# xiaojino/RUArt

Hardware: AMD Instinct MI355X
Metric: VQA samples/sec fwd+bwd (B=64, q=30, ocr=100) (higher is better)
Workload: dtype f16 MFMA + block-scaled fp8 (e4m3) MFMA correction, f32 accumulate / residual stream; 1 GPU; RUArt training step, synthetic ST-VQA-shaped batch: B=64/GPU, q=30 words, 100 OCR items, 36 objects, bert-base 12x768 frozen, SDNet trunk fwd+bwd, Adamax; global_batch=64, real_wordpieces_per_batch=42738, parallelism=dp1, mode=train

## Files before the change

### ruart_amd/bert.py

```python
import ctypes
import os
from ctypes import c_void_p

import numpy as np
import torch
import torch.nn as nn

from . import hip

LONG_BLOCK = 128
ROW_PAD = 256


def _np(x):
    return x.detach().cpu().numpy() if isinstance(x, torch.Tensor) else np.asarray(x)


def split_f16c(x, lo_shift=None, hi_shift=None):
    hi = x.to(torch.float16)
    lo = x - hi.to(torch.float32)
    sa_lo, sa_hi, _, _ = hip.f16c_shifts()
    lo_shift = sa_lo if lo_shift is None else lo_shift
    hi_shift = sa_hi if hi_shift is None else hi_shift
    pair = torch.cat([lo * float(2.0 ** lo_shift), x * float(2.0 ** hi_shift)], 1).clamp_(-448.0, 448.0)
# ... 137 lines not shown


def train_layer_split(opt, n_layers):
    if "bert_train_layers" not in opt:
        return 0
    n = opt["bert_train_layers"]
    if isinstance(n, bool) or not isinstance(n, (int, np.integer)) or n < 1 or n > n_layers:
        raise ValueError("opt['bert_train_layers'] = %r: the number of trained top layers is an integer in 1 .. %d" % (n, n_layers))
    if "LOCK_BERT" in opt:
        raise ValueError("opt['bert_train_layers'] trains encoder layers, LOCK_BERT freezes all of them: a conf has one or the other")
    if str(opt.get("bert_train_gemm", "x3")) != "16":
        raise ValueError("opt['bert_train_layers'] cuts the 16-bit trainable encoder only: it needs opt['bert_train_gemm'] = '16' (got %r)"
                         % (opt.get("bert_train_gemm", "x3"),))
    if opt.get("bert_no_pack", False):
        raise ValueError("opt['bert_train_layers'] runs on the packed token stream: it does not combine with opt['bert_no_pack']")
    return int(n_layers) - int(n)


class LowerLayers:

    def __init__(self, weights, k):
        if not 0 < k <= weights.n_layers:
            raise ValueError("the lower part holds 1 .. %d layers, not %d" % (weights.n_layers, k))
        self.full = weights
        self.cfg, self.device, self.precision = weights.cfg, weights.device, weights.precision
        self.dtype, self.tdtype, self.corr8, self.ln_fold = weights.dtype, weights.tdtype, weights.corr8, weights.ln_fold
        self.hidden, self.n_layers = weights.hidden, int(k)
        m = hip.BertModelC()
        ctypes.memmove(ctypes.byref(m), ctypes.byref(weights.c_model), ctypes.sizeof(m))
        m.n_layers = int(k)
        self.c_model = m
        if self.ln_fold:
            self.ln2_g_all, self.ln2_b_all = weights.ln2_g_all[:k], weights.ln2_b_all[:k]


class PackedTokens:

    def __init__(self, groups, device=None, pack=True, mfma_long=True, window=512, max_positions=None, dedup=False):
        ids_l, pos_l, len_l, bias_l = [], [], [], []
        self.group_index = []
        base = 0
        for ids, mask in groups:
            ids = _np(ids).astype(np.int64)
            mask = _np(mask).astype(bool)
            N, L = ids.shape
            if max_positions is not None and min(L, window) > max_positions:
                raise ValueError("BERT input rows of %d word pieces need %d position embeddings, the checkpoint has %d"
                                 % (L, min(L, window), max_positions))
            keep = mask if pack else np.ones_like(mask)
            if (keep.sum(1) == 0).any():
                raise ValueError("a BERT input row has no attendable token")
            nw = (L + window - 1) // window
            canon = None
            if dedup and nw == 1 and N > 1:
                key = np.ascontiguousarray(np.where(keep, ids, -1))
                _, first, inv = np.unique(key.view(np.dtype((np.void, key.dtype.itemsize * L))).reshape(-1), return_index=True, return_inverse=True)
                canon = first[inv.reshape(-1)]
                if (canon == np.arange(N)).all():
                    canon = None
                else:
                    keep = keep & (canon == np.arange(N))[:, None]
            if nw == 1:
                lens = keep.sum(1).astype(np.int64)
                lens = lens[lens > 0] if canon is not None else lens
            else:
                padded = np.zeros((N, nw * window), dtype=bool)
                padded[:, :L] = keep
                lens = padded.reshape(N, nw, window).sum(2).reshape(-1).astype(np.int64)
                lens = lens[lens > 0]
            flat = keep.reshape(-1)
            idx = np.full(N * L, -1, dtype=np.int64)
            idx[flat] = base + np.arange(int(flat.sum()))
            idx = idx.reshape(N, L)
            self.group_index.append(idx if canon is None else idx[canon])
            ids_l.append(ids.reshape(-1)[flat])
            pos_l.append(np.broadcast_to(np.arange(L) % window, (N, L)).reshape(-1)[flat])
            len_l.append(lens)
            if not pack:
                bias_l.append(np.where(mask.reshape(-1), 0.0, -10000.0).astype(np.float32))
            base += int(flat.sum())
        lens = np.concatenate(len_l)
        T = int(lens.sum())
        Tp = (T + ROW_PAD - 1) // ROW_PAD * ROW_PAD
        cu = np.zeros(len(lens) + 1, dtype=np.int64)
        np.cumsum(lens, out=cu[1:])
        seq_of = np.repeat(np.arange(len(lens)), lens)
        blk, lblk = self._plan_blocks(lens, cu, mfma_long)
        nb, nlb = blk.shape[1], lblk.shape[1]
        host = np.zeros(2 * Tp + 2 * T + 4 * nb + 4 * nlb, dtype=np.int32)
        host[0:T] = np.concatenate(ids_l)
        host[Tp:Tp + T] = np.concatenate(pos_l)
        host[2 * Tp:2 * Tp + T] = cu[seq_of]
        host[2 * Tp + T:2 * Tp + 2 * T] = cu[seq_of + 1]
        host[2 * Tp + 2 * T:2 * Tp + 2 * T + 4 * nb] = blk.reshape(-1)
        host[2 * Tp + 2 * T + 4 * nb:] = lblk.reshape(-1)
        self.T, self.Tp, self.n_blocks, self.n_long_blocks = T, Tp, nb, nlb
        self.n_seq = len(lens)
        self.max_len = int(lens.max())
        self.max_pos = int(host[Tp:Tp + T].max()) + 1 if T else 0
        self.sum_len_sq = float((lens.astype(np.float64) ** 2).sum())
        self.host = host
        self.bias_host = np.concatenate(bias_l) if not pack else None
        self.buf = None
        if device is not None:
            self.bind(device)

    _DEVICE_FIELDS = ("buf", "ids", "pos", "tok_lo", "tok_hi", "blk", "lblk", "key_bias", "c_batch", "_layers", "_event", "_set", "_train_plan",
                      "_emb_sorts", "last_rows")

    def prepare_embedding_sorts(self):
        if getattr(self, "_emb_sorts_host", None) is None:
            from .batch import _sort_ids
            T, Tp = self.T, self.Tp
            sorts = [_sort_ids(ids) for ids in (self.host[0:T], self.host[Tp:Tp + T])]
            self._emb_sorts_host = (np.concatenate([a for srt in sorts for a in srt]).astype(np.int32), [[len(a) for a in srt] for srt in sorts])
        return self._emb_sorts_host

    def train_plan(self, device):
        plan = getattr(self, "_train_plan", None)
        if plan is None or plan["device"] != device:
            T, Tp, nb, nlb = self.T, self.Tp, self.n_blocks, self.n_long_blocks
            o = 2 * Tp + 2 * T
            blk = self.host[o:o + 4 * nb].reshape(4, nb)
            lblk = self.host[o + 4 * nb:o + 4 * nb + 4 * nlb].reshape(4, nlb)
            own = (blk[0] == blk[2]) & (blk[1] == blk[3]) & ((blk[1] - blk[0]) <= 64)
            win = blk[:2, own]
            ch = [tuple(int(v) for v in blk[:, i]) for i in np.nonzero(~own)[0]]
            for i in range(nlb):
                q0, q1, k0, k1 = (int(v) for v in lblk[:, i])
                ch += [(a, min(a + 64, q1), k0, k1) for a in range(q0, q1, 64)]
            ch.sort()
            ok = all(q1 - q0 <= 64 and (q0 - k0) % 64 == 0 and k0 <= q0 < q1 <= k1 for q0, q1, k0, k1 in ch)
            idx = {c[0]: i for i, c in enumerate(ch)}
            ok = ok and all(k0 in idx and (q0 - k0) // 64 == i - idx[k0] for i, (q0, q1, k0, k1) in enumerate(ch))
            arr = np.array([c + (idx.get(c[2], 0),) for c in ch], dtype=np.int32).reshape(-1, 5).T.copy()
            both = torch.from_numpy(np.concatenate([win.reshape(-1), arr.reshape(-1)]).astype(np.int32)).to(device)
            nw, nc = win.shape[1], arr.shape[1]
            plan = {"device": device, "ok": bool(ok), "n_win": nw, "n_chunks": nc,
                    "win": [both[i * nw:(i + 1) * nw] for i in range(2)],
                    "chunks": [both[2 * nw + i * nc:2 * nw + (i + 1) * nc] for i in range(5)]}
            self._train_plan = plan
        return plan

    def embedding_sorts(self, device):
        if getattr(self, "_emb_sorts", None) is None:
            flat, sizes = self.prepare_embedding_sorts()
            dev = torch.from_numpy(flat).to(device, non_blocking=True)
            out, o = [], 0
            for group in sizes:
                views = []
                for n in group:
                    views.append(dev[o:o + n])
                    o += n
                out.append(tuple(views))
            self._emb_sorts = out
        return self._emb_sorts

    def __getstate__(self):
        return {k: v for k, v in self.__dict__.items() if k not in self._DEVICE_FIELDS}

    def __setstate__(self, state):
        self.__dict__.update(state)
        self.buf = None

    def bind(self, device, host_tensor=None):
        T, Tp, nb, nlb = self.T, self.Tp, self.n_blocks, self.n_long_blocks
        dev = (host_tensor if host_tensor is not None else torch.from_numpy(self.host)).to(device, non_blocking=True)
        self.buf = dev
        o = 0
        self.ids = dev[o:o + Tp]; o += Tp
        self.pos = dev[o:o + Tp]; o += Tp
        self.tok_lo = dev[o:o + T]; o += T
        self.tok_hi = dev[o:o + T]; o += T
        self.blk = [dev[o + i * nb:o + (i + 1) * nb] for i in range(4)]
        o += 4 * nb
        self.lblk = [dev[o + i * nlb:o + (i + 1) * nlb] for i in range(4)]
        self.key_bias = None
        if self.bias_host is not None:
            self.key_bias = torch.from_numpy(self.bias_host).to(device)
        b = hip.BertBatchC()
        b.n_tokens, b.n_rows, b.n_blocks = T, Tp, nb
        b.ids, b.pos_ids = self.ids.data_ptr(), self.pos.data_ptr()
        b.blk_q0, b.blk_q1, b.blk_k0, b.blk_k1 = [t.data_ptr() for t in self.blk]
        b.tok_lo, b.tok_hi = self.tok_lo.data_ptr(), self.tok_hi.data_ptr()
        b.key_bias = self.key_bias.data_ptr() if self.key_bias is not None else None
        b.n_long_blocks = nlb
        b.lblk_q0, b.lblk_q1, b.lblk_k0, b.lblk_k1 = [t.data_ptr() if nlb else None for t in self.lblk]
        b.n_last_rows, b.last_rows = 0, None
        self.c_batch = b
        return self

    def set_last_rows(self, rows_dev):
        self.last_rows = rows_dev
        self.c_batch.n_last_rows = int(rows_dev.numel())
        self.c_batch.last_rows = rows_dev.data_ptr()

    @staticmethod
    def _plan_blocks(lens, cu, mfma_long=True):
        S = len(lens)
        short, long_ = [], []
        s = 0
        while s < S:
            if lens[s] > 64:
                tgt, step = (long_, LONG_BLOCK) if mfma_long else (short, 64)
                for q0 in range(int(cu[s]), int(cu[s + 1]), step):
                    tgt.append((q0, min(q0 + step, int(cu[s + 1])), int(cu[s]), int(cu[s + 1])))
                s += 1
                continue
            e = int(np.searchsorted(cu, cu[s] + 64, side="right")) - 1
            while e > s + 1 and (lens[s:e] > 64).any():
                e -= 1
            e = max(e, s + 1)
            short.append((int(cu[s]), int(cu[e]), int(cu[s]), int(cu[e])))
            s = e
        def arr(x):
            return np.array(x, dtype=np.int32).reshape(-1, 4).T.copy()
        return arr(short), arr(long_)


class _Buffers:

    def __init__(self):
        self.layers = None
        self.ws = None
        self.stats = None

    def get(self, w, Tp):
        lib = hip.kernels()
        es = 4 if w.dtype == hip.DT_F32 else 2
        need_l = w.n_layers * Tp * w.hidden * es
        if self.layers is None or self.layers.numel() < need_l or self.layers.device != w.device:
            self.layers = torch.zeros(need_l, dtype=torch.uint8, device=w.device)
        fold = getattr(w, "ln_fold", False)
        need_w = int((lib.ruart_bert_workspace_bytes_folded if fold else lib.ruart_bert_workspace_bytes)(ctypes.byref(w.c_model), Tp))
        if self.ws is None or self.ws.numel() < need_w or self.ws.device != w.device:
            self.ws = torch.zeros(need_w, dtype=torch.uint8, device=w.device)
        if fold:
            need_s = w.n_layers * Tp * 2
            if self.stats is None or self.stats.numel() < need_s or self.stats.device != w.device:
                self.stats = torch.zeros(need_s, dtype=torch.float32, device=w.device)
        return self.layers[:need_l].view(w.tdtype).view(w.n_layers, Tp, w.hidden), self.ws, need_w

    def stats_for(self, w, Tp):
        return self.stats[:w.n_layers * Tp * 2].view(w.n_layers, Tp, 2)


_buffers = _Buffers()


def bert_encode(weights, packed, buffers=None):
    lib = hip.kernels()
    if getattr(packed, "max_pos", 0) > weights.cfg["max_position_embeddings"]:
        raise ValueError("the packed stream addresses %d position embeddings, the checkpoint has %d"
                         % (packed.max_pos, weights.cfg["max_position_embeddings"]))
    buffers = buffers or _buffers
    layers, ws, ws_bytes = buffers.get(weights, packed.Tp)
    if getattr(weights, "ln_fold", False):
        stats = buffers.stats_for(weights, packed.Tp)
        lib.ruart_bert_forward_folded(ctypes.byref(weights.c_model), ctypes.byref(packed.c_batch), layers, stats, ws, ws_bytes, hip.stream_ptr())
        layers._ln = (stats, weights.ln2_g_all, weights.ln2_b_all)
        return layers
    lib.ruart_bert_forward(ctypes.byref(weights.c_model), ctypes.byref(packed.c_batch), layers, ws, ws_bytes, hip.stream_ptr())
    return layers


def layer_outputs(layers, n_last=None):
    ln = getattr(layers, "_ln", None)
    if ln is None:
        return layers
    stats, g, b = ln
    return (layers - stats[:, :, 0:1]) * stats[:, :, 1:2] * g[:, None, :] + b[:, None, :]


from .ops import _ABL_SKIP


class _PoolMix(torch.autograd.Function):

    @staticmethod
    def forward(ctx, layer_w, layers, span_start, span_len, dst_row, n_rows, dtype_code, span_start_last=None, ln_stats=None, ln_g=None,
                ln_b=None):
        lib = hip.kernels()
        NL, Tp, H = layers.shape
        W = span_start.numel()
        out = torch.zeros(n_rows, H, dtype=torch.float32, device=layers.device)
        lw = layer_w.detach().to(torch.float32).contiguous()
        if W > 0 and "pool" not in _ABL_SKIP:
            if ln_stats is not None:
                lib.ruart_bert_pool_mix_ln(layers, Tp * H, H, NL, ln_stats, Tp, ln_g, ln_b, span_start, span_start_last, span_len, dst_row, lw,
                                           out, H, W, H, hip.stream_ptr())
            else:
                lib.ruart_bert_pool_mix(layers, Tp * H, H, dtype_code, NL, span_start, span_start_last, span_len, dst_row, lw, out, H, W, H,
                                        hip.stream_ptr())
        ctx.save_for_backward(layers, span_start, span_len, dst_row, span_start_last, ln_stats, ln_g, ln_b)
        ctx.dtype_code = dtype_code
        return out

    @staticmethod
    def backward(ctx, grad_out):
        lib = hip.kernels()
        layers, span_start, span_len, dst_row, span_start_last, ln_stats, ln_g, ln_b = ctx.saved_tensors
        NL, Tp, H = layers.shape
        W = span_start.numel()
        g = torch.zeros(NL, dtype=torch.float32, device=layers.device)
        if W > 0 and "pool" not in _ABL_SKIP:
            grad_out = grad_out.contiguous()
            partial = torch.empty(W * NL, dtype=torch.float32, device=layers.device)
            if ln_stats is not None:
                lib.ruart_bert_pool_mix_ln_bwd(layers, Tp * H, H, NL, ln_stats, Tp, ln_g, ln_b, span_start, span_start_last, span_len, dst_row,
                                               grad_out, H, partial, g, W, H, hip.stream_ptr())
            else:
                lib.ruart_bert_pool_mix_bwd(layers, Tp * H, H, ctx.dtype_code, NL, span_start, span_start_last, span_len, dst_row, grad_out, H,
                                            partial, g, W, H, hip.stream_ptr())
        return g, None, None, None, None, None, None, None, None, None, None


def word_spans(packed, group, offsets, word_mask, offsets_arr=None):
    wm = _np(word_mask).astype(bool)
    N, Lw = wm.shape
    if offsets_arr is None:
        offsets_arr = np.zeros((N, Lw, 2), dtype=np.int64)
        for n, row in enumerate(offsets):
            if len(row) and not isinstance(row[0], (list, tuple)):
                continue
            k = min(len(row), Lw)
            if k:
                offsets_arr[n, :k] = np.asarray(row[:k], dtype=np.int64)
    offsets_arr = _np(offsets_arr)
    st, ed = offsets_arr[..., 0], offsets_arr[..., 1]
    sel = wm & (ed > st)
    n_idx, j_idx = np.nonzero(sel)
    gidx = packed.group_index[group]
    s, e = st[sel], ed[sel]
    start = gidx[n_idx, s]
    last = gidx[n_idx, e - 1]
    if (start < 0).any() or (last - start != e - s - 1).any():
        raise ValueError("a word's piece span touches a masked BERT position; encode this batch with pack=False")
    return start.astype(np.int32), (e - s).astype(np.int32), (n_idx * Lw + j_idx).astype(np.int32), N * Lw


class Bert(nn.Module):

    def __init__(self, opt, device=None):
        super().__init__()
        import json
        import os
        self.opt = opt
        self.linear_combine = "BERT_LINEAR_COMBINE" in opt
        self.bert_dim, self.bert_layer = (1024, 24) if "BERT_LARGE" in opt else (768, 12)
        self._device = torch.device(device if device is not None else "cuda")
        if "bert_state" in opt:
            state, cfg = opt["bert_state"], opt["bert_config"]
        else:
            key = "BERT_large_model_file" if "BERT_LARGE" in opt else "BERT_model_file"
            d = os.path.join(opt.get("datadir", ""), opt[key])
            with open(os.path.join(d, "bert_config.json")) as f:
                cfg = json.load(f)
            state = torch.load(os.path.join(d, "pytorch_model.bin"), map_location="cpu")
        if cfg["hidden_size"] != self.bert_dim or cfg["num_hidden_layers"] != self.bert_layer:
            raise ValueError("BERT checkpoint is %dx%d, conf expects %dx%d" % (cfg["num_hidden_layers"], cfg["hidden_size"],
                                                                              self.bert_layer, self.bert_dim))
        from . import precision_of
        precision = precision_of(opt, cfg["hidden_size"] if cfg["intermediate_size"] % 256 == 0 else 1)
        fold = bool(int(opt.get("bert_ln_fold", os.environ.get("RUART_LN_FOLD", 1))))
        if int(opt.get("bert_tail_cus", os.environ.get("RUART_TAIL_CUS", 0)) or 0) > 0:
            fold = False
        if precision != "fp16c":
            fold = False
        self.weights = BertEncoderWeights(state, cfg, self._device, precision, ln_fold=fold)
        self.n_frozen = train_layer_split(opt, cfg["num_hidden_layers"])
        self.bert_model = None
        self._source = (state, cfg)
        self.pack = not opt.get("bert_no_pack", False)
        self._opt_prefetch_cus = opt.get("bert_prefetch_cus", 224 if precision == "fp16c" else 0)
        self._init_pipeline()
        tail = opt.get("bert_tail_cus", os.environ.get("RUART_TAIL_CUS", 0))
        self.weights.c_model.tail_cus = max(0, int(tail))

    def unlock(self):
        from .bert_train import BertModelTrainable
        if not self.pack:
            raise NotImplementedError("the trainable encoder runs on the packed token stream (bert_no_pack is for the frozen path)")
        state, cfg = self._source
        mode = str(self.opt.get("bert_train_gemm", "x3"))
        if mode == "16" and cfg["hidden_size"] % 256 == 0 and cfg["intermediate_size"] % 256 == 0:
            from .bert_train16 import BertModelTrainable16
            self.bert_model = BertModelTrainable16(state, cfg, self._device)
            self.bert_model.accurate_forward = bool(self.opt.get("bert_train_accurate_fwd", True))
            if self.n_frozen and self.weights.precision != "fp16c":
                raise ValueError("opt['bert_train_layers']: the frozen lower layers run on the fp16c kernels (bert_precision = %r)"
                                 % (self.weights.precision,))
            if self.n_frozen:
                self._lower_weights = LowerLayers(self.weights, self.n_frozen)
                self.bert_model.freeze_below(self.n_frozen, self.lower_layers_for)
        else:
            if self.n_frozen:
                raise ValueError("opt['bert_train_layers'] needs hidden / intermediate sizes that are multiples of 256")
            self.bert_model = BertModelTrainable(state, cfg, self._device, gemm="16" if mode in ("16", "16gemm") else "x3")
        self._source = None

    def lock(self):
        if self.opt.get("bert_frozen_dropout"):
            from .bert_train import BertModelTrainable
            state, cfg = self._source
            if (self.weights.precision in ("fp16c", "fp16", "bf16") and cfg["hidden_size"] % 256 == 0
                    and cfg["intermediate_size"] % 256 == 0):
                from .bert_train16 import BertModelTrainable16
                model = BertModelTrainable16(state, cfg, self._device)
            else:
                model = BertModelTrainable(state, cfg, self._device, gemm="x3")
            for p in model.parameters():
                p.requires_grad_(False)
            self.__dict__["_dropout_model"] = model
        self._source = None

    def _frozen_dropout_active(self):
        return self.training and self.__dict__.get("_dropout_model") is not None

    def _init_pipeline(self):
        self._bufsets = [_Buffers(), _Buffers()]
        self._pending = None
        self._in_use = 1
        cus = os.environ.get("RUART_PREFETCH_CUS", self._opt_prefetch_cus)
        self._pf_cus = cus if cus == "auto" else int(cus)
        self._pf_streams = {}

    def plan_prefetch_cus(self, n_rows):
        cfg = self.weights.cfg
        H, I = cfg["hidden_size"], cfg["intermediate_size"]
        rt = -(-int(n_rows) // 256)
        prods = ((3 * H // 256, 1.0), (H // 256, 1.0), (I // 256, 1.0), (H // 256, I / float(H)))
        best = None
        for c in range(208, 249, 8):
            cost = sum(w * -(-rt * nt // c) for nt, w in prods)
            if best is None or cost < best[0] - 1e-9:
                best = (cost, c)
        return best[1]

    def prefetch_cus(self, packed=None):
        if self.training:
            if self._pf_cus == "auto":
                if packed is None:
                    return 240
                self._pf_cus = self.plan_prefetch_cus(packed.Tp)
            return self._pf_cus
        return int(os.environ.get("RUART_PREFETCH_CUS_EVAL", 0))

    def prefetch(self, packed, after_stream=None):
        lower = self.runs_ahead()
        if getattr(packed, "_layers", None) is not None or (getattr(self, "bert_model", None) is not None and not lower) \
                or self._frozen_dropout_active():
            return
        weights = self._lower_weights if lower else self.weights
        dev = self._device
        cus = self.prefetch_cus(packed)
        st = self._pf_streams.get(cus)
        if st is None or st.device != dev:
            epr = int(os.environ.get("RUART_ENCODER_PRIORITY", 0))
            st = self._pf_streams[cus] = hip.cu_masked_stream(cus, dev) if cus > 0 else torch.cuda.Stream(device=dev, priority=epr)
        if after_stream is not None:
            st.wait_stream(after_stream)
        elif getattr(self, "_pickup_event", None) is not None:
            st.wait_event(self._pickup_event)
        else:
            st.wait_stream(torch.cuda.current_stream(dev))
        if getattr(self, "_last_pf_event", None) is not None:
            st.wait_event(self._last_pf_event)
        if self._pending is not None and self._pending is not packed:
            self._pending._layers = None
        self._pending = packed
        with torch.cuda.stream(st):
            packed._set = self._in_use ^ 1
            packed._layers = bert_encode(weights, packed, self._bufsets[packed._set])
            packed._event = self._last_pf_event = st.record_event()

    def close(self, destroy=None):
        if destroy is None:
            destroy = os.environ.get("RUART_DESTROY_STREAMS") == "1"
        if self._pending is not None:
            self._pending._layers = None
            self._pending = None
        if not destroy:
            for st in getattr(self, "_pf_streams", {}).values():
                st.synchronize()
            return
        streams, self._pf_streams = getattr(self, "_pf_streams", {}), {}
        self._last_pf_event = None
        for st in streams.values():
            hip.destroy_stream(st)

    def layers_for(self, packed):
        if getattr(self, "bert_model", None) is not None:
            return self.bert_model(packed, training=self.training)
        if self._frozen_dropout_active():
            with torch.no_grad():
                model = self.__dict__["_dropout_model"]
                fast = model.layers_nograd(packed, training=True) if hasattr(model, "layers_nograd") else None
                return fast if fast is not None else model(packed, training=True)
        return self._pickup(packed, self.weights)

    def runs_ahead(self):
        model = getattr(self, "bert_model", None)
        return bool(model is not None and self.n_frozen and self.training and self.opt.get("bert_train_prefetch", True)
                    and model.mixed_pass(True))

    def lower_layers_for(self, packed):
        return self._pickup(packed, self._lower_weights)

    def _pickup(self, packed, weights):
        layers = getattr(packed, "_layers", None)
        if layers is not None:
            torch.cuda.current_stream(self._device).wait_event(packed._event)
            packed._layers = None
            self._pending = None
            self._in_use = packed._set
            self._pickup_event = torch.cuda.current_stream(self._device).record_event()
            return layers
        pend = self._pending
        if pend is None or getattr(pend, "_layers", None) is None or pend._set != self._in_use ^ 1:
            self._in_use ^= 1
        self._pickup_event = torch.cuda.current_stream(self._device).record_event()
        return bert_encode(weights, packed, self._bufsets[self._in_use])

    def encode(self, groups):
        packed = PackedTokens(groups, self._device, pack=self.pack, mfma_long=self.weights.dtype != hip.DT_F32,
                              max_positions=self.weights.cfg["max_position_embeddings"])
        if getattr(self, "bert_model", None) is not None:
            return packed, self.bert_model(packed, training=self.training)
        return packed, bert_encode(self.weights, packed)

    def pool_mix(self, packed, layers, group, offsets, word_mask, layer_w, offsets_arr=None):
        s, n, d, rows = word_spans(packed, group, offsets, word_mask, offsets_arr)
        dev = self._device
        desc = torch.from_numpy(np.concatenate([s, n, d])).to(dev)
        W = len(s)
        if getattr(self, "bert_model", None) is not None:
            from .bert_train import pool_mix
            out = pool_mix(layer_w, layers, desc[:W], desc[W:2 * W], desc[2 * W:], rows)
        else:
            ln = getattr(layers, "_ln", None) or (None, None, None)
            out = _PoolMix.apply(layer_w, layers, desc[:W], desc[W:2 * W], desc[2 * W:], rows, hip.dtype_code(layers), None, *ln)
        N, Lw = word_mask.shape
        return out.view(N, Lw, self.weights.hidden)

    def forward(self, x_bert, x_bert_mask, x_bert_offset, x_mask, device=None):
        bs = getattr(self, "opt", {}).get("BERT_MAX_BatchSize")
        N = x_bert.shape[0]
        if bs and N > bs:
            parts = []
            for st in range(0, N, int(bs)):
                ed = min(st + int(bs), N)
                off = x_bert_offset[st:ed] if x_bert_offset is not None else None
                parts.append(self.forward(x_bert[st:ed], x_bert_mask[st:ed], off, x_mask[st:ed], device=device))
            return [torch.cat([p[i] for p in parts], 0) for i in range(len(parts[0]))]
        packed, layers = self.encode([(x_bert, x_bert_mask)])
        outs = []
        eye = torch.eye(self.weights.n_layers, device=self._device)
        for l in range(self.weights.n_layers):
            outs.append(self.pool_mix(packed, layers, 0, x_bert_offset, x_mask, eye[l]))
        return outs
```

### ruart_amd/csrc/bert_kernels.hip

```cpp
#include <stdlib.h>
#include "common.h"
#include <type_traits>
#include "ruart_hip.h"

#define MAXG 4

template <typename TOut>
struct RowStorePlain {
  TOut* out;
  __device__ __forceinline__ void operator()(int c, f32x4_t o) const { store4(out + c, o); }
};
struct RowStoreSplit {
  float* o32;
  f16_t* o16;
  unsigned char* o8;
  int H;
  __device__ __forceinline__ void operator()(int c, f32x4_t o) const {
    store4(o32 + c, o);
    store_split4(o16 + c, o8 + c, H, o);
  }
};

template <typename Store>
__device__ __forceinline__ void ln_row_finish(f32x4_t (&v)[MAXG], int H, int lane, const float* gamma, const float* beta,
// ... 1098 lines not shown
  g_attn_split_hpg = heads_per_workgroup;
  return 0;
}

extern "C" int ruart_bert_embed_ln(const int* ids, const int* pos, const float* word_emb, const float* pos_emb,
                                   const float* type_emb, const float* gamma, const float* beta, float eps, void* out, int ldo,
                                   int out_dtype, int rows, int H, void* stream) {
  RUART_ENTRY();
  if (H % 4 || H > 256 * MAXG || rows <= 0 || (ldo & 3)) return (int)hipErrorInvalidValue;
  const dim3 grid(ceil_div(rows, 4)), block(256);
  if (out_dtype == RUART_DT_BF16)
    hipLaunchKernelGGL(embed_ln_kernel<bf16_t>, grid, block, 0, (hipStream_t)stream, ids, pos, word_emb, pos_emb, type_emb, gamma, beta, eps, (bf16_t*)out, ldo, rows, H);
  else if (out_dtype == RUART_DT_F16)
    hipLaunchKernelGGL(embed_ln_kernel<f16_t>, grid, block, 0, (hipStream_t)stream, ids, pos, word_emb, pos_emb, type_emb, gamma, beta, eps, (f16_t*)out, ldo, rows, H);
  else
    hipLaunchKernelGGL(embed_ln_kernel<float>, grid, block, 0, (hipStream_t)stream, ids, pos, word_emb, pos_emb, type_emb, gamma, beta, eps, (float*)out, ldo, rows, H);
  RUART_CHECK_LAUNCH();
  return 0;
}

extern "C" int ruart_bert_attention(const void* qkv, int ld, void* ctx, int ldc, int dtype, int H, int n_heads, int n_blocks,
                                    const int* blk_q0, const int* blk_q1, const int* blk_k0, const int* blk_k1,
                                    const int* tok_lo, const int* tok_hi, const float* key_bias, int n_long_blocks,
                                    const int* lblk_q0, const int* lblk_q1, const int* lblk_k0, const int* lblk_k1, void* stream) {
  RUART_ENTRY();
  if (n_heads * 64 != H || n_blocks < 0 || n_long_blocks < 0 || n_blocks + n_long_blocks <= 0) return (int)hipErrorInvalidValue;
  if (n_long_blocks > 0 && dtype == RUART_DT_F32) return (int)hipErrorInvalidValue;
  hipStream_t st = (hipStream_t)stream;
  if (dtype == RUART_DT_F32) {
    if (n_blocks > 0) {
      hipLaunchKernelGGL(attn_varlen_kernel<float>, dim3(n_blocks, n_heads), dim3(64), 0, st, (const float*)qkv, ld, (float*)ctx, ldc, H, blk_q0, blk_q1, blk_k0, blk_k1, tok_lo, tok_hi, key_bias);
      RUART_CHECK_LAUNCH();
    }
    return 0;
  }
  if (n_blocks > 0) {
    const dim3 grid = attn_grid(n_blocks, n_heads), block(256);
    if (dtype == RUART_DT_BF16)
      hipLaunchKernelGGL(attn_flash_kernel<bf16_t>, grid, block, 0, st, (const bf16_t*)qkv, ld, (bf16_t*)ctx, ldc, H, blk_q0, blk_q1, blk_k0, blk_k1, tok_lo, key_bias);
    else
      hipLaunchKernelGGL(attn_flash_kernel<f16_t>, grid, block, 0, st, (const f16_t*)qkv, ld, (f16_t*)ctx, ldc, H, blk_q0, blk_q1, blk_k0, blk_k1, tok_lo, key_bias);
    RUART_CHECK_LAUNCH();
  }
  if (n_long_blocks > 0) {
    const dim3 grid = attn_grid(n_long_blocks, n_heads), block(256);
    if (dtype == RUART_DT_BF16)
      hipLaunchKernelGGL(attn_flash_long_kernel<bf16_t>, grid, block, 0, st, (const bf16_t*)qkv, ld, (bf16_t*)ctx, ldc, H, lblk_q0, lblk_q1, lblk_k0, lblk_k1, key_bias, n_long_blocks);
    else
      hipLaunchKernelGGL(attn_flash_long_kernel<f16_t>, grid, block, 0, st, (const f16_t*)qkv, ld, (f16_t*)ctx, ldc, H, lblk_q0, lblk_q1, lblk_k0, lblk_k1, key_bias, n_long_blocks);
    RUART_CHECK_LAUNCH();
  }
  return 0;
}

struct PoolLN {
  const float2* stats;
  size_t stats_stride;
  const float* g;
  const float* b;
};
__global__ __launch_bounds__(256) void pool_mix_cols_ln_kernel(const float* __restrict__ layers, size_t layer_stride, int ldl, int NL,
                                                               const int* __restrict__ span_start, const int* __restrict__ span_start_last,
                                                               const int* __restrict__ span_len, const int* __restrict__ dst_row,
                                                               const float* __restrict__ wl, float* __restrict__ out, int ldo, int W, int H,
                                                               PoolLN ln) {
  constexpr int LB = 6;
  const int w = blockIdx.x;
  const int st = span_start[w], n = span_len[w];
  const int st_last = span_start_last ? span_start_last[w] : st;
  const float inv = 1.0f / (float)n;
  const int col = threadIdx.x * 4;
  f32x4_t acc = {0.f, 0.f, 0.f, 0.f};
  auto body = [&](auto two_tag) {
    constexpr bool TWO = decltype(two_tag)::value;
    for (int lb = 0; lb < NL; lb += LB) {
      f32x4_t v[LB][TWO ? 2 : 1], g[LB], be[LB];
      float2 sa[LB][TWO ? 2 : 1];
      float wgt[LB];
#pragma unroll
      for (int j = 0; j < LB; ++j) {
        const int l = min(lb + j, NL - 1);
        wgt[j] = (lb + j < NL) ? wl[l] : 0.f;
        const int r0 = (l == NL - 1 ? st_last : st);
        const float* base = layers + (size_t)l * layer_stride + (size_t)r0 * ldl + col;
        v[j][0] = load4_stream(base);
        sa[j][0] = ln.stats[(size_t)l * ln.stats_stride + r0];
        if (TWO) {
          v[j][TWO ? 1 : 0] = load4_stream(base + (size_t)ldl);
          sa[j][TWO ? 1 : 0] = ln.stats[(size_t)l * ln.stats_stride + r0 + 1];
        }
        g[j] = load4(ln.g + (size_t)l * H + col);
        be[j] = load4(ln.b + (size_t)l * H + col);
      }
#pragma unroll
      for (int j = 0; j < LB; ++j) {
        f32x4_t x;
#pragma unroll
        for (int r = 0; r < 4; ++r) {
          x[r] = (v[j][0][r] - sa[j][0].x) * sa[j][0].y;
          if (TWO) x[r] += (v[j][TWO ? 1 : 0][r] - sa[j][TWO ? 1 : 0].x) * sa[j][TWO ? 1 : 0].y;
        }
        acc += (x * g[j]) * (wgt[j] * inv) + be[j] * wgt[j];
      }
      if (TWO && n > 2) {
        for (int j = 0; j < LB && lb + j < NL; ++j) {
          const int r0 = (lb + j == NL - 1 ? st_last : st);
          const float* base = layers + (size_t)(lb + j) * layer_stride + (size_t)r0 * ldl + col;
          for (int p = 2; p < n; ++p) {
            const float2 s2 = ln.stats[(size_t)(lb + j) * ln.stats_stride + r0 + p];
            const f32x4_t y = load4_stream(base + (size_t)p * ldl);
            f32x4_t x;
#pragma unroll
            for (int r = 0; r < 4; ++r) x[r] = (y[r] - s2.x) * s2.y;
            acc += (x * g[j]) * (wgt[j] * inv);
          }
        }
      }
    }
  };
  if (n > 1) body(std::true_type{});
  else body(std::false_type{});
  store4(out + (size_t)dst_row[w] * ldo + col, acc);
}

#define RUART_POOL_LN_WPB 4
template <int NLT>
__global__ __launch_bounds__(256) void pool_mix_cols_ln_reg_kernel(const float* __restrict__ layers, size_t layer_stride, int ldl,
                                                                   const int* __restrict__ span_start, const int* __restrict__ span_start_last,
                                                                   const int* __restrict__ span_len, const int* __restrict__ dst_row,
                                                                   const float* __restrict__ wl, float* __restrict__ out, int ldo, int W, int H,
                                                                   PoolLN ln) {
  constexpr int LB = 6, WPB = RUART_POOL_LN_WPB;
  static_assert(NLT % LB == 0, "layers are loaded six at a time");
  const int col = threadIdx.x * 4;
  f32x4_t g[NLT], be[NLT];
  float wgt[NLT];
  f32x4_t bsum = {0.f, 0.f, 0.f, 0.f};
#pragma unroll
  for (int l = 0; l < NLT; ++l) {
    g[l] = load4(ln.g + (size_t)l * H + col);
    be[l] = load4(ln.b + (size_t)l * H + col);
    wgt[l] = wl[l];
    bsum += be[l] * wgt[l];
  }
  for (int wi = 0; wi < WPB; ++wi) {
    const int w = blockIdx.x * WPB + wi;
    if (w >= W) break;
    const int st = span_start[w], n = span_len[w];
    const int st_last = span_start_last ? span_start_last[w] : st;
    const float inv = 1.0f / (float)n;
    f32x4_t acc = bsum;
    auto stat_of = [&](int l, int p) { return ln.stats[(size_t)l * ln.stats_stride + (l == NLT - 1 ? st_last : st) + min(p, n - 1)]; };
    auto body = [&](auto two_tag) {
      constexpr bool TWO = decltype(two_tag)::value;
#pragma unroll
      for (int lb = 0; lb < NLT; lb += LB) {
        f32x4_t v[LB][TWO ? 2 : 1];
#pragma unroll
        for (int j = 0; j < LB; ++j) {
          const int l = lb + j;
          const int r0 = (l == NLT - 1 ? st_last : st);
          const float* base = layers + (size_t)l * layer_stride + (size_t)r0 * ldl + col;
          v[j][0] = load4_stream(base);
          if (TWO) v[j][TWO ? 1 : 0] = load4_stream(base + (size_t)ldl);
        }
#pragma unroll
        for (int j = 0; j < LB; ++j) {
          const float2 s0 = stat_of(lb + j, 0), s1 = stat_of(lb + j, TWO ? 1 : 0);
          f32x4_t x;
#pragma unroll
          for (int r = 0; r < 4; ++r) {
            x[r] = (v[j][0][r] - s0.x) * s0.y;
            if (TWO) x[r] += (v[j][TWO ? 1 : 0][r] - s1.x) * s1.y;
          }
          acc += (x * g[lb + j]) * (wgt[lb + j] * inv);
        }
        if (TWO && n > 2) {
#pragma unroll
          for (int j = 0; j < LB; ++j) {
            const int r0 = (lb + j == NLT - 1 ? st_last : st);
            const float* base = layers + (size_t)(lb + j) * layer_stride + (size_t)r0 * ldl + col;
            for (int p = 2; p < n; ++p) {
              const float2 s2 = ln.stats[(size_t)(lb + j) * ln.stats_stride + r0 + p];
              const f32x4_t y = load4_stream(base + (size_t)p * ldl);
              f32x4_t x;
#pragma unroll
              for (int r = 0; r < 4; ++r) x[r] = (y[r] - s2.x) * s2.y;
              acc += (x * g[lb + j]) * (wgt[lb + j] * inv);
            }
          }
        }
      }
    };
    if (n > 1) body(std::true_type{});
    else body(std::false_type{});
    store4(out + (size_t)dst_row[w] * ldo + col, acc);
  }
}

template <int NG>
__global__ __launch_bounds__(256) void pool_mix_bwd_ln_kernel(const float* __restrict__ layers, size_t layer_stride, int ldl, int NL,
                                                              const int* __restrict__ span_start, const int* __restrict__ span_start_last,
                                                              const int* __restrict__ span_len, const int* __restrict__ dst_row,
                                                              const float* __restrict__ gout, int ldg, float* __restrict__ partial, int W, int H,
                                                              PoolLN ln) {
  const int lane = threadIdx.x & 63, wv = threadIdx.x >> 6;
  const int w = blockIdx.x;
  const int st = span_start[w], n = span_len[w];
  const int st_last = span_start_last ? span_start_last[w] : st;
  const float inv = 1.0f / (float)n;
  const int per = (NL + 3) >> 2;
  const int l0 = wv * per, l1 = min(NL, l0 + per);
  f32x4_t gv[NG];
  int col[NG];
  const float* g = gout + (size_t)dst_row[w] * ldg;
#pragma unroll
  for (int i = 0; i < NG; ++i) {
    col[i] = (i * 64 + lane) * 4;
    gv[i] = load4(g + col[i]);
  }
  for (int l = l0; l < l1; ++l) {
    const int r0 = (l == NL - 1 ? st_last : st);
    const float* base = layers + (size_t)l * layer_stride + (size_t)r0 * ldl;
    f32x4_t x[NG];
#pragma unroll
    for (int i = 0; i < NG; ++i) x[i] = (f32x4_t){0.f, 0.f, 0.f, 0.f};
    for (int p = 0; p < n; ++p) {
      const float2 s2 = ln.stats[(size_t)l * ln.stats_stride + r0 + p];
#pragma unroll
      for (int i = 0; i < NG; ++i) {
        const f32x4_t y = load4_stream(base + (size_t)p * ldl + col[i]);
#pragma unroll
        for (int r = 0; r < 4; ++r) x[i][r] += (y[r] - s2.x) * s2.y;
      }
    }
    f32x4_t s4 = {0.f, 0.f, 0.f, 0.f};
#pragma unroll
    for (int i = 0; i < NG; ++i) {
      const f32x4_t gg = load4(ln.g + (size_t)l * H + col[i]), bb = load4(ln.b + (size_t)l * H + col[i]);
      s4 += ((x[i] * gg) * inv + bb) * gv[i];
    }
    const float d = wave_sum((s4[0] + s4[1]) + (s4[2] + s4[3]));
    if (lane == 0) partial[(size_t)w * NL + l] = d;
  }
}

template <int NG, int NLT>
__global__ __launch_bounds__(256) void pool_mix_bwd_ln_reg_kernel(const float* __restrict__ layers, size_t layer_stride, int ldl,
                                                                  const int* __restrict__ span_start, const int* __restrict__ span_start_last,
                                                                  const int* __restrict__ span_len, const int* __restrict__ dst_row,
                                                                  const float* __restrict__ gout, int ldg, float* __restrict__ partial, int W, int H,
                                                                  PoolLN ln) {
  constexpr int PER = NLT / 4, WPB = RUART_POOL_LN_WPB;
  static_assert(NLT % 4 == 0, "the four waves share the layers evenly");
  const int lane = threadIdx.x & 63, wv = threadIdx.x >> 6;
  const int l0 = wv * PER;
  f32x4_t gg[PER][NG], bb[PER][NG];
  int col[NG];
#pragma unroll
  for (int i = 0; i < NG; ++i) col[i] = (i * 64 + lane) * 4;
#pragma unroll
  for (int k = 0; k < PER; ++k)
#pragma unroll
    for (int i = 0; i < NG; ++i) {
      gg[k][i] = load4(ln.g + (size_t)(l0 + k) * H + col[i]);
      bb[k][i] = load4(ln.b + (size_t)(l0 + k) * H + col[i]);
    }
  for (int wi = 0; wi < WPB; ++wi) {
    const int w = blockIdx.x * WPB + wi;
    if (w >= W) break;
    const int st = span_start[w], n = span_len[w];
    const int st_last = span_start_last ? span_start_last[w] : st;
    const float inv = 1.0f / (float)n;
    f32x4_t gv[NG];
    const float* g = gout + (size_t)dst_row[w] * ldg;
#pragma unroll
    for (int i = 0; i < NG; ++i) gv[i] = load4(g + col[i]);
#pragma unroll
    for (int k = 0; k < PER; ++k) {
      const int l = l0 + k;
      const int r0 = (l == NLT - 1 ? st_last : st);
      const float* base = layers + (size_t)l * layer_stride + (size_t)r0 * ldl;
      f32x4_t x[NG];
#pragma unroll
      for (int i = 0; i < NG; ++i) x[i] = (f32x4_t){0.f, 0.f, 0.f, 0.f};
      for (int p = 0; p < n; ++p) {
        const float2 s2 = ln.stats[(size_t)l * ln.stats_stride + r0 + p];
#pragma unroll
        for (int i = 0; i < NG; ++i) {
          const f32x4_t y = load4_stream(base + (size_t)p * ldl + col[i]);
#pragma unroll
          for (int r = 0; r < 4; ++r) x[i][r] += (y[r] - s2.x) * s2.y;
        }
      }
      f32x4_t s4 = {0.f, 0.f, 0.f, 0.f};
#pragma unroll
      for (int i = 0; i < NG; ++i) s4 += ((x[i] * gg[k][i]) * inv + bb[k][i]) * gv[i];
      const float d = wave_sum((s4[0] + s4[1]) + (s4[2] + s4[3]));
      if (lane == 0) partial[(size_t)w * NLT + l] = d;
    }
  }
}

__global__ __launch_bounds__(256) void rows_stats_finish_kernel(const float* __restrict__ part, int np, int rows, float inv_h, float eps,
                                                                float2* __restrict__ stats) {
  const int r = blockIdx.x * 256 + threadIdx.x;
  if (r >= rows) return;
  const f32x4_t a = load4(part + (size_t)r * 8), b = load4(part + (size_t)r * 8 + 4);
  const float ps[4] = {a[0], a[2], b[0], b[2]}, pq[4] = {a[1], a[3], b[1], b[3]};
  float s = 0.f, q = 0.f;
#pragma unroll
  for (int k = 0; k < 4; ++k)
    if (k < np) {
      s += ps[k];
      q += pq[k];
    }
  const float mu = s * inv_h;
  const float var = fmaxf(q * inv_h - mu * mu, 0.f);
  stats[r] = make_float2(mu, 1.0f / sqrtf(var + eps));
}
extern "C" int ruart_rows_stats_finish(const float* part, int np, int rows, float inv_h, float eps, float* stats, void* stream) {
  RUART_ENTRY();
  if (!part || !stats || np <= 0 || np > 4 || rows <= 0) return (int)hipErrorInvalidValue;
  hipLaunchKernelGGL(rows_stats_finish_kernel, dim3(ceil_div(rows, 256)), dim3(256), 0, (hipStream_t)stream, part, np, rows, inv_h, eps,
                     (float2*)stats);
  RUART_CHECK_LAUNCH();
  return 0;
}

static int g_pool_ln_reg = 1;
extern "C" int ruart_bert_pool_ln_set_variant(int reg_tables) {
  g_pool_ln_reg = reg_tables < 0 ? 0 : (reg_tables > 2 ? 2 : reg_tables);
  return 0;
}
extern "C" int ruart_bert_pool_mix_ln(const float* layers_pre, long long layer_stride, int ldl, int n_layers, const float* ln_stats,
                                      long long stats_stride, const float* ln_gamma, const float* ln_beta, const int* span_start,
                                      const int* span_start_last, const int* span_len, const int* dst_row, const float* layer_w, float* out,
                                      int ldo, int n_words, int H, void* stream) {
  RUART_ENTRY();
  if (H % 256 || H <= 0 || H > 1024 || n_words <= 0 || n_layers > POOL_MAX_LAYERS || n_layers <= 0 || !ln_stats || !ln_gamma || !ln_beta)
    return (int)hipErrorInvalidValue;
  const PoolLN ln{(const float2*)ln_stats, (size_t)stats_stride, ln_gamma, ln_beta};
  if (n_layers == 12 && g_pool_ln_reg)
    hipLaunchKernelGGL(pool_mix_cols_ln_reg_kernel<12>, dim3(ceil_div(n_words, RUART_POOL_LN_WPB)), dim3(H / 4), 0, (hipStream_t)stream, layers_pre,
                       (size_t)layer_stride, ldl, span_start, span_start_last, span_len, dst_row, layer_w, out, ldo, n_words, H, ln);
  else
    hipLaunchKernelGGL(pool_mix_cols_ln_kernel, dim3(n_words), dim3(H / 4), 0, (hipStream_t)stream, layers_pre, (size_t)layer_stride, ldl, n_layers,
                       span_start, span_start_last, span_len, dst_row, layer_w, out, ldo, n_words, H, ln);
  RUART_CHECK_LAUNCH();
  return 0;
}

extern "C" int ruart_bert_pool_mix_ln_bwd(const float* layers_pre, long long layer_stride, int ldl, int n_layers, const float* ln_stats,
                                          long long stats_stride, const float* ln_gamma, const float* ln_beta, const int* span_start,
                                          const int* span_start_last, const int* span_len, const int* dst_row, const float* grad_out, int ldg,
                                          float* partial_ws, float* grad_layer_w, int n_words, int H, void* stream) {
  RUART_ENTRY();
  if (H % 256 || H <= 0 || H > 1024 || n_words <= 0 || n_layers > POOL_MAX_LAYERS || n_layers <= 0 || !ln_stats || !ln_gamma || !ln_beta)
    return (int)hipErrorInvalidValue;
  const PoolLN ln{(const float2*)ln_stats, (size_t)stats_stride, ln_gamma, ln_beta};
  if (n_layers == 12 && H == 768 && g_pool_ln_reg == 2) {
    hipLaunchKernelGGL((pool_mix_bwd_ln_reg_kernel<3, 12>), dim3(ceil_div(n_words, RUART_POOL_LN_WPB)), dim3(256), 0, (hipStream_t)stream, layers_pre,
                       (size_t)layer_stride, ldl, span_start, span_start_last, span_len, dst_row, grad_out, ldg, partial_ws, n_words, H, ln);
  } else {
#define POOL(NG) hipLaunchKernelGGL((pool_mix_bwd_ln_kernel<NG>), dim3(n_words), dim3(256), 0, (hipStream_t)stream, layers_pre, (size_t)layer_stride, ldl, n_layers, span_start, span_start_last, span_len, dst_row, grad_out, ldg, partial_ws, n_words, H, ln)
    switch (H / 256) { case 1: POOL(1); break; case 2: POOL(2); break; case 3: POOL(3); break; default: POOL(4); }
#undef POOL
  }
  RUART_CHECK_LAUNCH();
  hipLaunchKernelGGL(reduce_partials_kernel, dim3(n_layers), dim3(256), 0, (hipStream_t)stream, partial_ws, n_words, n_layers, grad_layer_w);
  RUART_CHECK_LAUNCH();
  return 0;
}

static int g_pool_cols = 1;
extern "C" int ruart_bert_pool_set_variant(int cols) {
  g_pool_cols = cols ? 1 : 0;
  return 0;
}

template <typename T>
static void launch_pool(const void* layers, long long layer_stride, int ldl, int n_layers, const int* span_start, const int* span_start_last,
                        const int* span_len, const int* dst_row, const float* layer_w, float* out, int ldo, int n_words, int H, hipStream_t st) {
  const dim3 grid(n_words), block(256);
  if (H % 256 == 0 && g_pool_cols) {
    hipLaunchKernelGGL((pool_mix_cols_kernel<T>), grid, dim3(H / 4), 0, st, (const T*)layers, (size_t)layer_stride, ldl, n_layers, span_start,
                       span_start_last, span_len, dst_row, layer_w, out, ldo, n_words, H);
    return;
  }
#define POOL(NG) hipLaunchKernelGGL((pool_mix_kernel<T, NG>), grid, block, 0, st, (const T*)layers, (size_t)layer_stride, ldl, n_layers, span_start, span_start_last, span_len, dst_row, layer_w, out, ldo, n_words, H)
  switch ((H + 255) / 256) { case 1: POOL(1); break; case 2: POOL(2); break; case 3: POOL(3); break; default: POOL(4); }
#undef POOL
}
template <typename T>
static void launch_pool_bwd(const void* layers, long long layer_stride, int ldl, int n_layers, const int* span_start,
                            const int* span_start_last, const int* span_len, const int* dst_row, const float* grad_out, int ldg, float* partial, int n_words, int H, hipStream_t st) {
  const dim3 grid(n_words), block(256);
#define POOL(NG) hipLaunchKernelGGL((pool_mix_bwd_kernel<T, NG>), grid, block, 0, st, (const T*)layers, (size_t)layer_stride, ldl, n_layers, span_start, span_start_last, span_len, dst_row, grad_out, ldg, partial, n_words, H)
  switch ((H + 255) / 256) { case 1: POOL(1); break; case 2: POOL(2); break; case 3: POOL(3); break; default: POOL(4); }
#undef POOL
}

extern "C" int ruart_bert_pool_mix(const void* layers, long long layer_stride, int ldl, int dtype, int n_layers,
                                   const int* span_start, const int* span_start_last, const int* span_len, const int* dst_row,
                                   const float* layer_w, float* out, int ldo, int n_words, int H, void* stream) {
  RUART_ENTRY();
  if (H % 4 || H < 4 || H > 1024 || n_words <= 0 || n_layers > POOL_MAX_LAYERS || n_layers <= 0) return (int)hipErrorInvalidValue;
  if (dtype == RUART_DT_BF16)
    launch_pool<bf16_t>(layers, layer_stride, ldl, n_layers, span_start, span_start_last, span_len, dst_row, layer_w, out, ldo, n_words, H, (hipStream_t)stream);
  else if (dtype == RUART_DT_F16)
    launch_pool<f16_t>(layers, layer_stride, ldl, n_layers, span_start, span_start_last, span_len, dst_row, layer_w, out, ldo, n_words, H, (hipStream_t)stream);
  else
    launch_pool<float>(layers, layer_stride, ldl, n_layers, span_start, span_start_last, span_len, dst_row, layer_w, out, ldo, n_words, H, (hipStream_t)stream);
  RUART_CHECK_LAUNCH();
  return 0;
}

extern "C" int ruart_bert_pool_mix_bwd(const void* layers, long long layer_stride, int ldl, int dtype, int n_layers,
                                       const int* span_start, const int* span_start_last, const int* span_len, const int* dst_row,
                                       const float* grad_out, int ldg, float* partial_ws, float* grad_layer_w, int n_words, int H,
                                       void* stream) {
  RUART_ENTRY();
  if (H % 4 || H < 4 || H > 1024 || n_words <= 0 || n_layers > POOL_MAX_LAYERS || n_layers <= 0) return (int)hipErrorInvalidValue;
  if (dtype == RUART_DT_BF16)
    launch_pool_bwd<bf16_t>(layers, layer_stride, ldl, n_layers, span_start, span_start_last, span_len, dst_row, grad_out, ldg, partial_ws, n_words, H, (hipStream_t)stream);
  else if (dtype == RUART_DT_F16)
    launch_pool_bwd<f16_t>(layers, layer_stride, ldl, n_layers, span_start, span_start_last, span_len, dst_row, grad_out, ldg, partial_ws, n_words, H, (hipStream_t)stream);
  else
    launch_pool_bwd<float>(layers, layer_stride, ldl, n_layers, span_start, span_start_last, span_len, dst_row, grad_out, ldg, partial_ws, n_words, H, (hipStream_t)stream);
  RUART_CHECK_LAUNCH();
  hipLaunchKernelGGL(reduce_partials_kernel, dim3(n_layers), dim3(256), 0, (hipStream_t)stream, partial_ws, n_words, n_layers, grad_layer_w);
  RUART_CHECK_LAUNCH();
  return 0;
}

struct GatherArgs {
  const char* src[3];
  char* dst[3];
  long long sp[3], dp[3];
  int bytes[3];
};
__global__ __launch_bounds__(256) void rows_gather_kernel(const int* __restrict__ rows, GatherArgs a) {
  const int i = blockIdx.x, r = rows[i];
#pragma unroll
  for (int k = 0; k < 3; ++k) {
    if (!a.src[k]) break;
    const char* s = a.src[k] + (size_t)r * a.sp[k];
    char* d = a.dst[k] + (size_t)i * a.dp[k];
    for (int o = threadIdx.x * 16; o < a.bytes[k]; o += 256 * 16) *reinterpret_cast<f32x4_t*>(d + o) = *reinterpret_cast<const f32x4_t*>(s + o);
  }
}

extern "C" int ruart_rows_gather(const int* rows, int n, const void* src0, long long sp0, void* dst0, long long dp0, int bytes0, const void* src1,
                                 long long sp1, void* dst1, long long dp1, int bytes1, const void* src2, long long sp2, void* dst2, long long dp2,
                                 int bytes2, void* stream) {
  RUART_ENTRY();
  if (!rows || n <= 0 || !src0 || !dst0) return (int)hipErrorInvalidValue;
  GatherArgs a;
  const void* src[3] = {src0, src1, src2};
  void* dst[3] = {dst0, dst1, dst2};
  const long long sp[3] = {sp0, sp1, sp2}, dp[3] = {dp0, dp1, dp2};
  const int by[3] = {bytes0, bytes1, bytes2};
  for (int k = 0; k < 3; ++k) {
    a.src[k] = (const char*)src[k];
    a.dst[k] = (char*)dst[k];
    a.sp[k] = sp[k];
    a.dp[k] = dp[k];
    a.bytes[k] = by[k];
    if (src[k] && (!dst[k] || by[k] <= 0 || (by[k] & 15) || (sp[k] & 15) || (dp[k] & 15) || ((uintptr_t)src[k] & 15) || ((uintptr_t)dst[k] & 15)))
      return (int)hipErrorInvalidValue;
  }
  hipLaunchKernelGGL(rows_gather_kernel, dim3(n), dim3(256), 0, (hipStream_t)stream, rows, a);
  RUART_CHECK_LAUNCH();
  return 0;
}

extern "C" int ruart_cast_f32_to_16(const float* in, void* out, int out_dtype, long long n, float scale, void* stream) {
  RUART_ENTRY();
  if (n % 4 || (out_dtype != RUART_DT_BF16 && out_dtype != RUART_DT_F16)) return (int)hipErrorInvalidValue;
  const size_t n4 = (size_t)n / 4;
  const int blocks = (int)((n4 + 255) / 256 < 2048 ? (n4 + 255) / 256 : 2048);
  if (out_dtype == RUART_DT_BF16)
    hipLaunchKernelGGL((cast_kernel<float, bf16_t>), dim3(blocks > 0 ? blocks : 1), dim3(256), 0, (hipStream_t)stream, in, (bf16_t*)out, n4, scale);
  else
    hipLaunchKernelGGL((cast_kernel<float, f16_t>), dim3(blocks > 0 ? blocks : 1), dim3(256), 0, (hipStream_t)stream, in, (f16_t*)out, n4, scale);
  RUART_CHECK_LAUNCH();
  return 0;
}
```

Baseline: 2880 samples/s.

## Add streaming double-buffered pool-mix LN backward kernel over word chunks

Adds a new backward kernel for the LayerNorm-fused layer-mix pooling that processes chunks of 4 words per block. It walks the subword rows with a cursor that prefetches the next word's metadata and double-buffers the layer-row loads, so memory latency overlaps with the FMA accumulation. Gamma/beta are applied once at the end from accumulated sums, and fewer partials go to the reduction. The Python side also skips the contiguous copy of grad_out when it is already aligned, and skips zero-filling the gradient buffer. It becomes the default path (variant 1) and carries more register pressure plus less parallelism per word.

```diff
diff --git a/ruart_amd/bert.py b/ruart_amd/bert.py
--- a/ruart_amd/bert.py
+++ b/ruart_amd/bert.py
@@ -463,16 +463,20 @@
         layers, span_start, span_len, dst_row, span_start_last, ln_stats, ln_g, ln_b = ctx.saved_tensors
         NL, Tp, H = layers.shape
         W = span_start.numel()
-        g = torch.zeros(NL, dtype=torch.float32, device=layers.device)
         if W > 0 and "pool" not in _ABL_SKIP:
-            grad_out = grad_out.contiguous()
+            if grad_out.stride(1) != 1 or grad_out.stride(0) % 4 or grad_out.data_ptr() % 16:
+                grad_out = grad_out.contiguous()
+            ldg = grad_out.stride(0)
+            g = torch.empty(NL, dtype=torch.float32, device=layers.device)
             partial = torch.empty(W * NL, dtype=torch.float32, device=layers.device)
             if ln_stats is not None:
                 lib.ruart_bert_pool_mix_ln_bwd(layers, Tp * H, H, NL, ln_stats, Tp, ln_g, ln_b, span_start, span_start_last, span_len, dst_row,
-                                               grad_out, H, partial, g, W, H, hip.stream_ptr())
+                                               grad_out, ldg, partial, g, W, H, hip.stream_ptr())
             else:
-                lib.ruart_bert_pool_mix_bwd(layers, Tp * H, H, ctx.dtype_code, NL, span_start, span_start_last, span_len, dst_row, grad_out, H,
+                lib.ruart_bert_pool_mix_bwd(layers, Tp * H, H, ctx.dtype_code, NL, span_start, span_start_last, span_len, dst_row, grad_out, ldg,
                                             partial, g, W, H, hip.stream_ptr())
+        else:
+            g = torch.zeros(NL, dtype=torch.float32, device=layers.device)
         return g, None, None, None, None, None, None, None, None, None, None
 
 
diff --git a/ruart_amd/csrc/bert_kernels.hip b/ruart_amd/csrc/bert_kernels.hip
--- a/ruart_amd/csrc/bert_kernels.hip
+++ b/ruart_amd/csrc/bert_kernels.hip
@@ -1424,6 +1424,150 @@
   }
 }
 
+struct PoolWord {
+  int st, stl, n, dst;
+};
+struct PoolCursor {
+  PoolWord cur, nxt;
+  int w, p;
+};
+__device__ __forceinline__ PoolWord pool_word(const int* __restrict__ span_start, const int* __restrict__ span_start_last,
+                                              const int* __restrict__ span_len, const int* __restrict__ dst_row, int w) {
+  PoolWord d;
+  d.st = span_start[w];
+  d.n = span_len[w];
+  d.stl = span_start_last[w];
+  d.dst = dst_row[w];
+  return d;
+}
+__device__ __forceinline__ PoolCursor pool_cursor(const int* __restrict__ span_start, const int* __restrict__ span_start_last,
+                                                  const int* __restrict__ span_len, const int* __restrict__ dst_row, int w0, int W) {
+  PoolCursor c;
+  c.w = w0;
+  c.p = 0;
+  c.cur = pool_word(span_start, span_start_last, span_len, dst_row, w0);
+  c.nxt = pool_word(span_start, span_start_last, span_len, dst_row, min(w0 + 1, W - 1));
+  return c;
+}
+__device__ __forceinline__ PoolCursor pool_advance(const PoolCursor& c, const int* __restrict__ span_start,
+                                                   const int* __restrict__ span_start_last, const int* __restrict__ span_len,
+                                                   const int* __restrict__ dst_row, int W) {
+  const PoolWord far = pool_word(span_start, span_start_last, span_len, dst_row, min(c.w + 2, W - 1));
+  const bool turn = c.p + 1 >= c.cur.n;
+  PoolCursor r;
+  r.w = turn ? c.w + 1 : c.w;
+  r.p = turn ? 0 : c.p + 1;
+  r.cur.st = turn ? c.nxt.st : c.cur.st;
+  r.cur.stl = turn ? c.nxt.stl : c.cur.stl;
+  r.cur.n = turn ? c.nxt.n : c.cur.n;
+  r.cur.dst = turn ? c.nxt.dst : c.cur.dst;
+  r.nxt.st = turn ? far.st : c.nxt.st;
+  r.nxt.stl = turn ? far.stl : c.nxt.stl;
+  r.nxt.n = turn ? far.n : c.nxt.n;
+  r.nxt.dst = turn ? far.dst : c.nxt.dst;
+  return r;
+}
+
+#define RUART_POOL_BWD_CHUNK 4
+template <int NG>
+__global__ __launch_bounds__(256) void pool_mix_bwd_ln_stream_kernel(const float* __restrict__ layers, size_t layer_stride, int ldl, int NL,
+                                                                     const int* __restrict__ span_start, const int* __restrict__ span_start_last,
+                                                                     const int* __restrict__ span_len, const int* __restrict__ dst_row,
+                                                                     const float* __restrict__ gout, int ldg, float* __restrict__ partial, int W,
+                                                                     int H, PoolLN ln) {
+  constexpr int CH = RUART_POOL_BWD_CHUNK, LP = POOL_LPB;
+  const int lane = threadIdx.x & 63;
+  const int wv = __builtin_amdgcn_readfirstlane(threadIdx.x >> 6);
+  const int per = (NL + 3) >> 2;
+  const int l0 = wv * per, l1 = min(NL, l0 + per);
+  const int w0 = blockIdx.x * CH, w_end = min(w0 + CH, W);
+  if (!span_start_last) span_start_last = span_start;
+  int col[NG];
+#pragma unroll
+  for (int i = 0; i < NG; ++i) col[i] = (i * 64 + lane) * 4;
+  struct Buf {
+    f32x4_t y[LP][NG], g[NG];
+    float2 s[LP];
+    float inv, first;
+  };
+  for (int lb = l0; lb < l1; lb += LP) {
+    int lay[LP];
+#pragma unroll
+    for (int j = 0; j < LP; ++j) lay[j] = min(lb + j, l1 - 1);
+    f32x4_t S[LP][NG], G[NG];
+#pragma unroll
+    for (int i = 0; i < NG; ++i) {
+      G[i] = (f32x4_t){0.f, 0.f, 0.f, 0.f};
+#pragma unroll
+      for (int j = 0; j < LP; ++j) S[j][i] = (f32x4_t){0.f, 0.f, 0.f, 0.f};
+    }
+    auto issue = [&](Buf& b, const PoolCursor& c) {
+#pragma unroll
+      for (int j = 0; j < LP; ++j) {
+        const size_t row = (size_t)((lay[j] == NL - 1 ? c.cur.stl : c.cur.st) + c.p);
+        const float* base = layers + (size_t)lay[j] * layer_stride + row * ldl;
+#pragma unroll
+        for (int i = 0; i < NG; ++i) b.y[j][i] = load4_stream(base + col[i]);
+        b.s[j] = ln.stats[(size_t)lay[j] * ln.stats_stride + row];
+      }
+      const float* g = gout + (size_t)c.cur.dst * ldg;
+#pragma unroll
+      for (int i = 0; i < NG; ++i) b.g[i] = load4(g + col[i]);
+      b.inv = 1.0f / (float)c.cur.n;
+      b.first = c.p == 0 ? 1.0f : 0.0f;
+    };
+    auto consume = [&](const Buf& b) {
+      f32x4_t gi[NG];
+#pragma unroll
+      for (int i = 0; i < NG; ++i) {
+        gi[i] = b.g[i] * b.inv;
+        G[i] += b.g[i] * b.first;
+      }
+#pragma unroll
+      for (int j = 0; j < LP; ++j) {
+        const float r = b.s[j].y, m = -b.s[j].x * r;
+#pragma unroll
+        for (int i = 0; i < NG; ++i)
+#pragma unroll
+          for (int k = 0; k < 4; ++k) S[j][i][k] = fmaf(fmaf(b.y[j][i][k], r, m), gi[i][k], S[j][i][k]);
+      }
+    };
+    Buf A, B;
+    PoolCursor c = pool_cursor(span_start, span_start_last, span_len, dst_row, w0, W);
+    issue(A, c);
+    for (;;) {
+      PoolCursor c2 = pool_advance(c, span_start, span_start_last, span_len, dst_row, W);
+      if (c2.w >= w_end) {
+        consume(A);
+        break;
+      }
+      issue(B, c2);
+      consume(A);
+      c = pool_advance(c2, span_start, span_start_last, span_len, dst_row, W);
+      if (c.w >= w_end) {
+        consume(B);
+        break;
+      }
+      issue(A, c);
+      consume(B);
+    }
+    float d[LP];
+#pragma unroll
+    for (int j = 0; j < LP; ++j) {
+      f32x4_t s4 = {0.f, 0.f, 0.f, 0.f};
+#pragma unroll
+      for (int i = 0; i < NG; ++i) {
+        const f32x4_t gg = load4(ln.g + (size_t)lay[j] * H + col[i]), bb = load4(ln.b + (size_t)lay[j] * H + col[i]);
+        s4 += S[j][i] * gg + G[i] * bb;
+      }
+      d[j] = wave_sum((s4[0] + s4[1]) + (s4[2] + s4[3]));
+    }
+#pragma unroll
+    for (int j = 0; j < LP; ++j)
+      if (lane == 0 && lb + j < l1) partial[(size_t)blockIdx.x * NL + lb + j] = d[j];
+  }
+}
+
 __global__ __launch_bounds__(256) void rows_stats_finish_kernel(const float* __restrict__ part, int np, int rows, float inv_h, float eps,
                                                                 float2* __restrict__ stats) {
   const int r = blockIdx.x * 256 + threadIdx.x;
@@ -1452,7 +1596,7 @@
 
 static int g_pool_ln_reg = 1;
 extern "C" int ruart_bert_pool_ln_set_variant(int reg_tables) {
-  g_pool_ln_reg = reg_tables < 0 ? 0 : (reg_tables > 2 ? 2 : reg_tables);
+  g_pool_ln_reg = reg_tables < 0 ? 0 : (reg_tables > 3 ? 3 : reg_tables);
   return 0;
 }
 extern "C" int ruart_bert_pool_mix_ln(const float* layers_pre, long long layer_stride, int ldl, int n_layers, const float* ln_stats,
@@ -1481,7 +1625,13 @@
   if (H % 256 || H <= 0 || H > 1024 || n_words <= 0 || n_layers > POOL_MAX_LAYERS || n_layers <= 0 || !ln_stats || !ln_gamma || !ln_beta)
     return (int)hipErrorInvalidValue;
   const PoolLN ln{(const float2*)ln_stats, (size_t)stats_stride, ln_gamma, ln_beta};
-  if (n_layers == 12 && H == 768 && g_pool_ln_reg == 2) {
+  int n_partial = n_words;
+  if (g_pool_ln_reg == 1) {
+    n_partial = ceil_div(n_words, RUART_POOL_BWD_CHUNK);
+#define POOL(NG) hipLaunchKernelGGL((pool_mix_bwd_ln_stream_kernel<NG>), dim3(n_partial), dim3(256), 0, (hipStream_t)stream, layers_pre, (size_t)layer_stride, ldl, n_layers, span_start, span_start_last, span_len, dst_row, grad_out, ldg, partial_ws, n_words, H, ln)
+    switch (H / 256) { case 1: POOL(1); break; case 2: POOL(2); break; case 3: POOL(3); break; default: POOL(4); }
+#undef POOL
+  } else if (n_layers == 12 && H == 768 && g_pool_ln_reg == 2) {
     hipLaunchKernelGGL((pool_mix_bwd_ln_reg_kernel<3, 12>), dim3(ceil_div(n_words, RUART_POOL_LN_WPB)), dim3(256), 0, (hipStream_t)stream, layers_pre,
                        (size_t)layer_stride, ldl, span_start, span_start_last, span_len, dst_row, grad_out, ldg, partial_ws, n_words, H, ln);
   } else {
@@ -1490,7 +1640,7 @@
 #undef POOL
   }
   RUART_CHECK_LAUNCH();
-  hipLaunchKernelGGL(reduce_partials_kernel, dim3(n_layers), dim3(256), 0, (hipStream_t)stream, partial_ws, n_words, n_layers, grad_layer_w);
+  hipLaunchKernelGGL(reduce_partials_kernel, dim3(n_layers), dim3(256), 0, (hipStream_t)stream, partial_ws, n_partial, n_layers, grad_layer_w);
   RUART_CHECK_LAUNCH();
   return 0;
 }
```

New measurement: 2885 samples/s (median of 6 runs). About the same (+0.2%).
